# smacke/ffsubsync

Measured on AMD Instinct MI355X. Metric: alignments/sec (2 h@100 Hz, 7 framerate ratios), higher is better.
Workload: dtype i32; 1 GPU; configs[2]: 8192 x 7200 s@100 Hz pairs per GPU (8 batches of 1024), MaxScoreAligner over 7 framerate ratios, max_offset_samples=6000; algorithm=auto, pairs_per_gpu=8192, pairs_in_flight=512, n_fft_reference=2097152, n_fft_device=786432, input_format=bit-packed 0/1 vectors (FFS_DTYPE_U1) resident in HBM, parallelism=single GPU

## Files before the change

ffsubsync_amd/csrc/ffs_runs.h:

```cpp
#pragma once
#include "ffs_kernels.h"

namespace ffsa {

#ifndef FFS_RUNS_THREADS
#define FFS_RUNS_THREADS 512
#define FFS_RUNS_T 12288
#define FFS_RUNS_QCAP 3070
#endif
constexpr int RUNS_THREADS = FFS_RUNS_THREADS;
constexpr int RUNS_WAVES = RUNS_THREADS / 64;
constexpr int RUNS_T = FFS_RUNS_T;
constexpr int RUNS_LPT = RUNS_T / RUNS_THREADS;
constexpr int RUNS_QCAP = FFS_RUNS_QCAP;
static_assert(RUNS_T % RUNS_THREADS == 0 && RUNS_LPT % 4 == 0 && RUNS_LPT <= 32, "whole groups of four lags per thread, 32-bit edge windows");
constexpr int RUNS_CAP = 32768;
#ifndef FFS_RUNS_TPW
#define FFS_RUNS_TPW 2
#endif
constexpr int RUNS_TPW = FFS_RUNS_TPW;
constexpr int RUNS_QSENT = 0x1fffffff;
static_assert(RUNS_LPT <= 32 && RUNS_LPT % 4 == 0 && RUNS_QCAP % 2 == 0, "one 32-bit mask per thread, 8-byte histogram loads");

struct RunsRef {
    const int2* e;
    const int2* hdr;
    const unsigned* bits;
    int32_t len;
    int32_t cap;
};

struct RunEntry {
    int pos, ones;
};
typedef const __attribute__((address_space(1))) RunEntry* GEntries;
typedef const __attribute__((address_space(1))) int* GInts;
typedef const __attribute__((address_space(1))) unsigned* GWords;

struct RunsBest {
    double score;
    int32_t d;
    int32_t pad;
};

struct PackVec {
    const unsigned char* src;
    unsigned* dst;
    int32_t len;
    int32_t pad;
};

__global__ __launch_bounds__(256) void k_pack_bytes_batch(const PackVec* __restrict__ vecs, int chunks_per_vec) {
    const int v = blockIdx.x / chunks_per_vec, c = blockIdx.x - v * chunks_per_vec;
    const PackVec pv = vecs[v];
    const long long n = pv.len;
    const long long w = (long long)c * 256 + threadIdx.x;
    const long long n_words = (n + 31) >> 5;
    if (w >= n_words) return;
    const long long i0 = w * 32;
    const unsigned char* __restrict__ p = pv.src + i0;
    unsigned out = 0;
    if (i0 + 32 <= n) {
        unsigned wd[8];
        __builtin_memcpy(wd, p, 32);
#pragma unroll
        for (int k = 0; k < 8; ++k) {
            const unsigned t = nz_flags(wd[k]) >> 7;
            out |= (((t * 0x00204081u) >> 21) & 0xfu) << (4 * k);
        }
    } else {
        for (int k = 0; k < 32 && i0 + k < n; ++k) out |= (unsigned)(p[k] != 0) << k;
    }
    pv.dst[w] = out;
}

FFS_HD bool runs_over_budget(long long n_p, long long n_q, long long cap_p, long long cap_q, long long W, long long R, long long budget) {
    if (n_p >= cap_p || n_q >= cap_q) return true;
    const long long pairs = n_p * n_q;
    return pairs * W / (R > 0 ? R : 1) > budget;
}

FFS_DEV unsigned wave_incl_scan_u32(unsigned v) {
#define FFS_DPP_ADD(ctrl, rows) v += (unsigned)__builtin_amdgcn_update_dpp(0, (int)v, ctrl, rows, 0xf, false)
    FFS_DPP_ADD(0x111, 0xf);
    FFS_DPP_ADD(0x112, 0xf);
    FFS_DPP_ADD(0x114, 0xf);
    FFS_DPP_ADD(0x118, 0xf);
    FFS_DPP_ADD(0x142, 0xa);
    FFS_DPP_ADD(0x143, 0xc);
#undef FFS_DPP_ADD
    return v;
}

FFS_DEV float wave_max_f32(float v) {
#define FFS_DPP_MAX(ctrl, rows) v = fmaxf(v, __int_as_float(__builtin_amdgcn_update_dpp(__float_as_int(v), __float_as_int(v), ctrl, rows, 0xf, false)))
    FFS_DPP_MAX(0x111, 0xf);
    FFS_DPP_MAX(0x112, 0xf);
    FFS_DPP_MAX(0x114, 0xf);
    FFS_DPP_MAX(0x118, 0xf);
    FFS_DPP_MAX(0x142, 0xa);
    FFS_DPP_MAX(0x143, 0xc);
#undef FFS_DPP_MAX
    return __int_as_float(__builtin_amdgcn_readlane(__float_as_int(v), 63));
}

constexpr int RUNS_XQ = 256;
template <int NT>
FFS_DEV void runs_extract_lds(unsigned (*&s_e)[NT / 64 * 2], unsigned (*&s_o)[NT / 64 * 2], uint4 (*&s_q)[RUNS_XQ]) {
    __shared__ unsigned l_e[2][NT / 64 * 2], l_o[2][NT / 64 * 2];
    __shared__ __attribute__((aligned(16))) uint4 l_q[NT / 64][RUNS_XQ];
    s_e = l_e, s_o = l_o, s_q = l_q;
}
template <int NT, bool compact = false>
FFS_DEV void runs_extract_body(const unsigned* __restrict__ w_generic, const int len, int2* __restrict__ e, int2* __restrict__ hdr,
                               const int cap) {
    constexpr int NWV = NT / 64;
    constexpr int G = 2, SWEEP = NT * 4 * G;
    const int tid = threadIdx.x, lane = tid & 63, wave = __builtin_amdgcn_readfirstlane(tid >> 6);
    const gptr eb = (gptr)e;
    const int nw = (len + 31) >> 5;
    const int n_proc = (len >> 5) + 1;
    const unsigned tail = (len & 31) ? ((1u << (len & 31)) - 1u) : 0xffffffffu;
    unsigned(*s_e)[NWV * 2], (*s_o)[NWV * 2];
    uint4(*s_q)[RUNS_XQ];
    runs_extract_lds<NT>(s_e, s_o, s_q);
    uint4* const ring = s_q[wave];
    unsigned q_head = 0, q_tail = 0;
    unsigned n_bound = 0, n_ones = 0;
    unsigned xn[G][4], pn[G];
    const __amdgpu_buffer_rsrc_t vrs = __builtin_amdgcn_make_buffer_rsrc(const_cast<unsigned*>(w_generic), 0, nw * 4, 0x00020000);
    auto request = [&](int base) {
#pragma unroll
        for (int g = 0; g < G; ++g) {
            const int w0 = base + (g * NT + tid) * 4;
            typedef unsigned v4u __attribute__((ext_vector_type(4)));
            const v4u t = __builtin_amdgcn_raw_buffer_load_b128(vrs, w0 * 4, 0, 2);
            xn[g][0] = t.x, xn[g][1] = t.y, xn[g][2] = t.z, xn[g][3] = t.w;
            pn[g] = 0;
            if (lane == 0) pn[g] = __builtin_amdgcn_raw_buffer_load_b32(vrs, w0 * 4 - 4, 0, 0);
        }
    };
    auto drain = [&]() {
        const unsigned n = (q_tail - q_head) < 64u ? (q_tail - q_head) : 64u;
        if ((unsigned)lane < n) {
            const uint4 it = ring[(q_head + (unsigned)lane) & (RUNS_XQ - 1)];
            unsigned eb_k = it.y ^ __builtin_amdgcn_alignbit(it.y, it.x, 31);
            const int pos0 = (int)((it.x & 0x7fffffffu) << 5);
            int k_out = (int)it.w;
            while (eb_k) {
                const int b = __builtin_ctz(eb_k);
                if (k_out < cap) {
                    typedef int v2i __attribute__((ext_vector_type(2)));
                    if (compact)
                        *(__attribute__((address_space(1))) int*)(eb + 4u * (unsigned)k_out) = pos0 + b;
                    else
                        *(__attribute__((address_space(1))) v2i*)(eb + 8u * (unsigned)k_out) =
                            (v2i){pos0 + b, (int)it.z + (int)__popc(it.y & ((1u << b) - 1u))};
                }
                ++k_out;
                eb_k &= eb_k - 1;
            }
        }
        q_head += n;
    };
    request(0);
    int buf = 0;
    for (int base = 0; base < n_proc && n_bound < (unsigned)cap; base += SWEEP, buf ^= 1) {
        unsigned x[G][4], pv[G];
#pragma unroll
        for (int g = 0; g < G; ++g) {
            pv[g] = pn[g];
#pragma unroll
            for (int k = 0; k < 4; ++k) x[g][k] = xn[g][k];
            const int w0 = base + (g * NT + tid) * 4;
            if ((unsigned)(nw - 1 - w0) < 4u) {
#pragma unroll
                for (int k = 0; k < 4; ++k)
                    if (w0 + k == nw - 1) x[g][k] &= tail;
            }
            if (w0 == nw) pv[g] &= tail;
        }
        while (q_tail - q_head >= 64u) drain();
        if (base + SWEEP < n_proc) request(base + SWEEP);
        unsigned ne[G], no[G], pc = 0;
        unsigned fr[G];
#pragma unroll
        for (int g = 0; g < G; ++g) {
            unsigned prev = (unsigned)__builtin_amdgcn_update_dpp(0, (int)x[g][3], 0x138, 0xf, 0xf, false);
            if (lane == 0) prev = pv[g];
            fr[g] = prev;
            unsigned nc = 0;
            ne[g] = no[g] = 0;
#pragma unroll
            for (int k = 0; k < 4; ++k) {
                const unsigned e_k = x[g][k] ^ __builtin_amdgcn_alignbit(x[g][k], prev, 31);
                prev = x[g][k];
                ne[g] += __popc(e_k);
                no[g] += __popc(x[g][k]);
                nc += e_k != 0u ? 1u : 0u;
            }
            pc |= nc << (16 * g);
        }
        const unsigned ic = wave_incl_scan_u32(pc);
        unsigned qe = 0, qo = 0, se = 0, so = 0;
        unsigned ie[G], io[G];
        if (NT <= 256) {
            static_assert(G == 2, "two groups per packed scan");
            const unsigned pe = ne[0] | (ne[1] << 16), po = no[0] | (no[1] << 16);
            const unsigned je = wave_incl_scan_u32(pe), jo = wave_incl_scan_u32(po);
            if (lane == 63) s_e[buf][wave] = je, s_o[buf][wave] = jo;
            __syncthreads();
            qe = je - pe, qo = jo - po;
#pragma unroll
            for (int i = 0; i < NWV; ++i) {
                const unsigned a = s_e[buf][i], b = s_o[buf][i];
                if (i < wave) qe += a, qo += b;
                se += a, so += b;
            }
        } else {
#pragma unroll
            for (int g = 0; g < G; ++g) {
                ie[g] = wave_incl_scan_u32(ne[g]), io[g] = wave_incl_scan_u32(no[g]);
                if (lane == 63) s_e[buf][wave * G + g] = ie[g], s_o[buf][wave * G + g] = io[g];
                ie[g] -= ne[g], io[g] -= no[g];
            }
            __syncthreads();
        }
        const unsigned wc = (unsigned)__builtin_amdgcn_readlane((int)ic, 63);
        const unsigned rc = ic - pc;
        unsigned gb = n_bound, go = n_ones;
#pragma unroll
        for (int g = 0; g < G; ++g) {
            unsigned xe_g, xo_g, te_g = 0, to_g = 0;
            if (NT <= 256) {
                xe_g = (qe >> (16 * g)) & 0xffffu, xo_g = (qo >> (16 * g)) & 0xffffu, te_g = (se >> (16 * g)) & 0xffffu, to_g = (so >> (16 * g)) & 0xffffu;
            } else {
                xe_g = ie[g], xo_g = io[g];
                for (int i = 0; i < NWV; ++i) {
                    const unsigned a = s_e[buf][i * G + g], b = s_o[buf][i * G + g];
                    if (i < wave) xe_g += a, xo_g += b;
                    te_g += a, to_g += b;
                }
            }
            unsigned k_out = gb + xe_g;
            unsigned ones = go + xo_g;
            gb += te_g;
            go += to_g;
            const unsigned add = (wc >> (16 * g)) & 0xffffu;
            {
            while (q_tail - q_head + add > (unsigned)RUNS_XQ) drain();
            unsigned slot = q_tail + ((rc >> (16 * g)) & 0xffffu);
            const unsigned w0 = (unsigned)(base + (g * NT + tid) * 4);
            unsigned prev = fr[g];
#pragma unroll
            for (int k = 0; k < 4; ++k) {
                const unsigned e_k = x[g][k] ^ __builtin_amdgcn_alignbit(x[g][k], prev, 31);
                if (e_k) {
                    ring[slot & (RUNS_XQ - 1)] = make_uint4((w0 + k) | (prev & 0x80000000u), x[g][k], ones, k_out);
                    ++slot;
                }
                k_out += __popc(e_k);
                ones += __popc(x[g][k]);
                prev = x[g][k];
            }
            q_tail += add;
            asm volatile("s_waitcnt lgkmcnt(0)" ::: "memory");
            }
        }
        n_bound = gb, n_ones = go;
    }
    while (q_tail != q_head) drain();
    if (tid == 0) {
        *hdr = make_int2((int)n_bound, (int)n_ones);
        if ((int)n_bound < cap) {
            if (compact)
                reinterpret_cast<int*>(e)[n_bound] = INT32_MAX;
            else
                e[n_bound] = make_int2(INT32_MAX, (int)n_ones);
        }
    }
}

constexpr int RUNS_PROBE_WORDS = 256;
__global__ __launch_bounds__(256) void k_runs_probe(const RunsRef* __restrict__ refs, int n_vec) {
    const int v = blockIdx.x * 4 + (threadIdx.x >> 6), lane = threadIdx.x & 63;
    if (v >= n_vec) return;
    const RunsRef r = refs[v];
    if (!r.bits) return;
    const GWords w = (GWords)r.bits;
    const int nw = r.len >> 5;
    unsigned cnt = 0;
    if (nw > 0) {
#pragma unroll
        for (int u = 0; u < RUNS_PROBE_WORDS / 64; ++u) {
            const long long k = ((long long)(u * 64 + lane) * nw) / RUNS_PROBE_WORDS;
            const unsigned x = w[k];
            cnt += __popc((x ^ (x << 1)) & 0xfffffffeu);
        }
    }
#pragma unroll
    for (int s = 32; s >= 1; s >>= 1) cnt += __shfl_xor(cnt, s, 64);
    if (lane == 0) {
        const long long sampled = (long long)(nw < RUNS_PROBE_WORDS ? (nw > 0 ? nw : 1) : RUNS_PROBE_WORDS) * 31;
        long long est = (long long)cnt * (long long)r.len / sampled;
        if (est > 0x3fffffff) est = 0x3fffffff;
        const_cast<int2*>(r.hdr)[0] = make_int2((int)est, 0);
    }
}

FFS_DEV void runs_extract_zero(int* __restrict__ zero, int zero_words) {
    if (zero && blockIdx.x == 0)
        for (int i = threadIdx.x; i < zero_words; i += blockDim.x) zero[i] = 0;
}
FFS_DEV bool runs_compact_vec(int cstride, int n_plain) {
    return cstride > 0 && (int)blockIdx.x < n_plain && (int)blockIdx.x % cstride != 0;
}
__global__ __launch_bounds__(256, 8) void k_runs_extract(const RunsRef* __restrict__ refs, int* __restrict__ zero, int zero_words,
                                                         int cstride, int n_plain) {
    runs_extract_zero(zero, zero_words);
    const RunsRef r = refs[blockIdx.x];
    if (!r.bits) return;
    if (runs_compact_vec(cstride, n_plain))
        runs_extract_body<256, true>(r.bits, r.len, const_cast<int2*>(r.e), const_cast<int2*>(r.hdr), r.cap);
    else
        runs_extract_body<256, false>(r.bits, r.len, const_cast<int2*>(r.e), const_cast<int2*>(r.hdr), r.cap);
}
__global__ __launch_bounds__(512, 4) void k_runs_extract_512(const RunsRef* __restrict__ refs, int with_len_cap, int* __restrict__ zero,
                                                             int zero_words, int cstride, int n_plain) {
    runs_extract_zero(zero, zero_words);
    const RunsRef r = refs[blockIdx.x];
    if (!r.bits) return;
    if (with_len_cap && threadIdx.x == 0) const_cast<int2*>(r.hdr)[1] = make_int2(r.len, r.cap);
    if (runs_compact_vec(cstride, n_plain))
        runs_extract_body<512, true>(r.bits, r.len, const_cast<int2*>(r.e), const_cast<int2*>(r.hdr), r.cap);
    else
        runs_extract_body<512, false>(r.bits, r.len, const_cast<int2*>(r.e), const_cast<int2*>(r.hdr), r.cap);
}
__global__ __launch_bounds__(1024, 4) void k_runs_extract_1024(const RunsRef* __restrict__ refs, int with_len_cap, int* __restrict__ zero,
                                                               int zero_words, int cstride, int n_plain) {
    runs_extract_zero(zero, zero_words);
    const RunsRef r = refs[blockIdx.x];
    if (!r.bits) return;
    if (with_len_cap && threadIdx.x == 0) const_cast<int2*>(r.hdr)[1] = make_int2(r.len, r.cap);
    if (runs_compact_vec(cstride, n_plain))
        runs_extract_body<1024, true>(r.bits, r.len, const_cast<int2*>(r.e), const_cast<int2*>(r.hdr), r.cap);
    else
        runs_extract_body<1024, false>(r.bits, r.len, const_cast<int2*>(r.e), const_cast<int2*>(r.hdr), r.cap);
}

__global__ __launch_bounds__(256, 8) void k_runs_extract_lists(const RunsRef* __restrict__ refs) {
    const RunsRef r = refs[blockIdx.x];
    if (threadIdx.x == 0) const_cast<int2*>(r.hdr)[1] = make_int2(r.len, r.cap);
    runs_extract_body<256>(r.bits, r.len, const_cast<int2*>(r.e), const_cast<int2*>(r.hdr), r.cap);
}

__global__ __launch_bounds__(1024, 4) void k_runs_extract_one(const unsigned* __restrict__ bits, int len, int2* __restrict__ e,
                                                             int2* __restrict__ hdr, int cap) {
    if (threadIdx.x == 0) hdr[1] = make_int2(len, cap);
    runs_extract_body<1024>(bits, len, e, hdr, cap);
}

static inline void runs_extract_launch(const RunsRef* refs, size_t n_vec, bool with_len_cap, hipStream_t st, int* zero = nullptr,
                                       int zero_words = 0, int cstride = 0, int n_plain = 0) {
    if (with_len_cap) cstride = 0;
    if (n_vec <= 256)
        hipLaunchKernelGGL(k_runs_extract_1024, dim3((unsigned)n_vec), dim3(1024), 0, st, refs, with_len_cap ? 1 : 0, zero, zero_words, cstride, n_plain);
    else if (n_vec <= 768)
        hipLaunchKernelGGL(k_runs_extract_512, dim3((unsigned)n_vec), dim3(512), 0, st, refs, with_len_cap ? 1 : 0, zero, zero_words, cstride, n_plain);
    else if (with_len_cap)
        hipLaunchKernelGGL(k_runs_extract_lists, dim3((unsigned)n_vec), dim3(256), 0, st, refs);
    else
        hipLaunchKernelGGL(k_runs_extract, dim3((unsigned)n_vec), dim3(256), 0, st, refs, zero, zero_words, cstride, n_plain);
}

FFS_DEV unsigned fetch32(GWords w, int len, long long start) {
    const int nw = (len + 31) >> 5;
    const long long wi = start >> 5;
    unsigned v[2];
#pragma unroll
    for (int k = 0; k < 2; ++k) {
        const long long i = wi + k;
        unsigned t = (i >= 0 && i < nw) ? w[i] : 0u;
        if (i == nw - 1 && (len & 31)) t &= (1u << (len & 31)) - 1u;
        v[k] = t;
    }
    return __builtin_amdgcn_alignbit(v[1], v[0], (unsigned)(start & 31));
}

FFS_DEV unsigned list_bits32(GEntries e, int n, long long start) {
    if (start + 32 <= 0 || n <= 0) return 0u;
    int lo = 0, hi = n;
    while (lo < hi) {
        const int mid = (lo + hi) >> 1;
        if ((long long)e[mid].pos <= start)
            lo = mid + 1;
        else
            hi = mid;
    }
    unsigned m = (lo & 1) ? 0xffffffffu : 0u;
    for (int k = lo; k < n; ++k) {
        const long long off = (long long)e[k].pos - start;
        if (off >= 32) break;
        m ^= 0xffffffffu << (int)off;
    }
    return m;
}

FFS_DEV int wave_lower_bound_e(GEntries a, int n, int x) {
    const int lane = threadIdx.x & 63;
    int lo = 0, len = n;
    while (len > 0) {
        const int step = (len + 63) >> 6;
        const int idx = lo + (lane + 1) * step - 1;
        const bool below = idx < lo + len && a[idx].pos < x;
        const int c = __popcll(__ballot(below));
        const int end = lo + len;
        lo += c * step;
        len = (step - 1) < (end - lo) ? (step - 1) : (end - lo);
    }
    return lo;
}

template <int NW>
FFS_DEV void block_excl_scan3(int& a, int& b, int& c, int* s_tmp) {
    const int lane = threadIdx.x & 63, wave = threadIdx.x >> 6;
    int ia = a, ib = b, ic = c;
#pragma unroll
    for (int s = 1; s < 64; s <<= 1) {
        const int oa = __shfl_up(ia, s, 64), ob = __shfl_up(ib, s, 64), oc = __shfl_up(ic, s, 64);
        if (lane >= s) ia += oa, ib += ob, ic += oc;
    }
    __syncthreads();
    if (lane == 63) s_tmp[wave * 3] = ia, s_tmp[wave * 3 + 1] = ib, s_tmp[wave * 3 + 2] = ic;
    __syncthreads();
    int pa = ia - a, pb = ib - b, pc = ic - c;
#pragma unroll
    for (int i = 0; i < NW - 1; ++i)
        if (i < wave) pa += s_tmp[i * 3], pb += s_tmp[i * 3 + 1], pc += s_tmp[i * 3 + 2];
    a = pa, b = pb, c = pc;
}

constexpr int RUNS_FLAG_SPLIT = 8;
static inline unsigned runs_flag_split(long long cands_per_chunk) {
    const long long want = (cands_per_chunk + 447) / 448;
    return (unsigned)(want < RUNS_FLAG_SPLIT ? RUNS_FLAG_SPLIT : (want > 128 ? 128 : want));
}
__global__ __launch_bounds__(256) void k_runs_chunk_flags(const CandDesc* __restrict__ cands, int n_pairs, int n_cand,
                                                          int pairs_per_chunk, const RunsRef* __restrict__ refs, long long budget,
                                                          int* __restrict__ flags, unsigned long long* __restrict__ stats,
                                                          int estimates) {
    const int ch = blockIdx.x;
    const int p0 = ch * pairs_per_chunk, p1 = (p0 + pairs_per_chunk) < n_pairs ? (p0 + pairs_per_chunk) : n_pairs;
    int over = 0, bad = 0;
    unsigned long long nb = 0;
    int longest = 0;
    for (int i = p0 * n_cand + (int)(blockIdx.y * 256 + threadIdx.x); i < p1 * n_cand; i += 256 * (int)gridDim.y) {
        const CandDesc& cd = cands[i];
        const int pair = i / n_cand, j = i - pair * n_cand;
        const int vr = pair * (n_cand + 1), vs = vr + 1 + j;
        const RunsRef rr = refs[vr], rs = refs[vs];
        const GInts hq = (GInts)rr.hdr, hp = (GInts)rs.hdr;
        const int n_q = hq[0], n_p = hp[0];
        const int cap_q = (estimates && rr.bits) ? 0x7fffffff : (rr.cap > 0 ? rr.cap : hq[3]);
        const int cap_p = (estimates && rs.bits) ? 0x7fffffff : (rs.cap > 0 ? rs.cap : hp[3]);
        nb += (unsigned)n_p + (j == 0 ? (unsigned)n_q : 0u);
        if (rs.bits && n_p > longest) longest = n_p;
        if (rr.bits && n_q > longest) longest = n_q;
        bad |= (!rs.bits && n_p >= cap_p) || (!rr.bits && n_q >= cap_q);
        if (cd.flags & CAND_NO_LAGS) continue;
        const int lim_q = (estimates && rr.bits) ? cap_q : (cap_q < RUNS_CAP ? cap_q : RUNS_CAP);
        const int lim_p = (estimates && rs.bits) ? cap_p : (cap_p < RUNS_CAP ? cap_p : RUNS_CAP);
        over |= runs_over_budget(n_p, n_q, lim_p, lim_q, (long long)cd.d_hi - cd.d_lo + 1, cd.R, budget) ? 1 : 0;
    }
    over = __syncthreads_or(over);
    bad = __syncthreads_or(bad);
    __shared__ unsigned long long s_nb[4];
#pragma unroll
    for (int s = 32; s >= 1; s >>= 1) nb += __shfl_xor(nb, s, 64);
    if ((threadIdx.x & 63) == 0) s_nb[threadIdx.x >> 6] = nb;
    __syncthreads();
    if (threadIdx.x == 0) {
        const int f = bad ? 2 : over;
        if (f) atomicMax(&flags[ch], f);
        if (!estimates) atomicAdd(stats, s_nb[0] + s_nb[1] + s_nb[2] + s_nb[3]);
    }
    if (!estimates) {
#pragma unroll
        for (int s = 32; s >= 1; s >>= 1) {
            const int o = __shfl_xor(longest, s, 64);
            longest = o > longest ? o : longest;
        }
        if ((threadIdx.x & 63) == 0 && longest > 0) atomicMax(stats + 1, (unsigned long long)longest);
    }
}

FFS_DEV void runs_write_cand(const CandDesc& cd, CandResult* __restrict__ cres, int ci, double score, int d, bool none) {
    CandResult r;
    if (none) {
        r.score = -INFINITY;
        r.offset = (long long)cd.n_ref - 1 - cd.S;
        r.score_f32 = -INFINITY;
        r.flags = 1;
    } else {
        r.score = score;
        r.offset = d;
        r.score_f32 = (float)score;
        r.flags = 0;
    }
    apply_zero_rule(cd, r);
    cres[ci] = r;
}

struct LevelInfo {
    double lam[4];
    double q;
    int32_t n_levels;
    int32_t m[3];
    int32_t ok;
    int32_t pad[3];
};
constexpr int LEVELS_MAX_MULT = 8;

template <class T>
FFS_DEV void levels_insert(double (&v)[5], int& n, T x) {
    const double d = (double)x;
    bool seen = false;
#pragma unroll
    for (int i = 0; i < 5; ++i) seen |= (i < n && v[i] == d);
    if (!seen && n < 5) {
#pragma unroll
        for (int i = 0; i < 5; ++i)
            if (i == n) v[i] = d;
        ++n;
    }
}

template <class T>
__global__ __launch_bounds__(256) void k_levels_sample(const T* const* __restrict__ vec, const int* __restrict__ len, LevelInfo* __restrict__ out) {
    const int v = blockIdx.x, tid = threadIdx.x, lane = tid & 63, wave = tid >> 6;
    typedef const __attribute__((address_space(1))) T* GT;
    const GT x = (GT)vec[v];
    const int n = len[v];
    double vals[5] = {0.0, 0.0, 0.0, 0.0, 0.0};
    int cnt = 0;
#pragma unroll
    for (int u = 0; u < 8; ++u) {
        const long long k = ((long long)(u * 256 + tid) * n) / 2048;
        if (k < n) levels_insert(vals, cnt, x[k]);
    }
    __shared__ double s_v[4][5];
    __shared__ int s_n[4];
    for (int s = 1; s < 64; s <<= 1) {
        const int cn = __shfl_xor(cnt, s, 64);
        double pv[5];
#pragma unroll
        for (int i = 0; i < 5; ++i) pv[i] = __shfl_xor(vals[i], s, 64);
#pragma unroll
        for (int i = 0; i < 5; ++i)
            if (i < cn) levels_insert(vals, cnt, pv[i]);
    }
    double (&wv)[5] = vals;
    const int wn = cnt;
    if (lane == 0) {
        s_n[wave] = wn;
#pragma unroll
        for (int i = 0; i < 5; ++i) s_v[wave][i] = wv[i];
    }
    __syncthreads();
    if (tid == 0) {
        double all[5];
        int an = 0;
        for (int w = 0; w < 4; ++w)
            for (int i = 0; i < s_n[w] && i < 5; ++i) levels_insert(all, an, s_v[w][i]);
        for (int i = 1; i < an && i < 5; ++i)
// ... 921 lines not shown
```

Before: 2.701 million 7-ratio solves/s.

## Stage run-boundary records in an LDS window and flush coalesced line-aligned stores

Boundary records produced by the run-extraction kernel are no longer written straight to global memory from the drain loop. Each sweep's records go into an LDS window, and the whole block then flushes them with line-aligned, coalesced stores at the start of the next sweep. The point is to replace scattered per-lane global writes with contiguous cache-line writes. The cost is extra LDS, a full queue drain every sweep, an extra synchronisation, and a fallback to direct stores when a sweep's records exceed the window. It also adds compile-time A/B switches for isolating store cost.

```diff
diff --git a/ffsubsync_amd/csrc/ffs_runs.h b/ffsubsync_amd/csrc/ffs_runs.h
--- a/ffsubsync_amd/csrc/ffs_runs.h
+++ b/ffsubsync_amd/csrc/ffs_runs.h
@@ -106,27 +106,38 @@
 
 constexpr int RUNS_XQ = 256;
 template <int NT>
-FFS_DEV void runs_extract_lds(unsigned (*&s_e)[NT / 64 * 2], unsigned (*&s_o)[NT / 64 * 2], uint4 (*&s_q)[RUNS_XQ]) {
+constexpr int runs_xwin_bytes() {
+    return NT == 256 ? 496 * 8 : NT * 16;
+}
+template <int NT>
+FFS_DEV void runs_extract_lds(unsigned (*&s_e)[NT / 64 * 2], unsigned (*&s_o)[NT / 64 * 2], uint4 (*&s_q)[RUNS_XQ], unsigned*& s_win) {
     __shared__ unsigned l_e[2][NT / 64 * 2], l_o[2][NT / 64 * 2];
     __shared__ __attribute__((aligned(16))) uint4 l_q[NT / 64][RUNS_XQ];
-    s_e = l_e, s_o = l_o, s_q = l_q;
+    __shared__ __attribute__((aligned(8))) unsigned l_win[runs_xwin_bytes<NT>() / 4];
+    s_e = l_e, s_o = l_o, s_q = l_q, s_win = l_win;
 }
 template <int NT, bool compact = false>
 FFS_DEV void runs_extract_body(const unsigned* __restrict__ w_generic, const int len, int2* __restrict__ e, int2* __restrict__ hdr,
                                const int cap) {
     constexpr int NWV = NT / 64;
     constexpr int G = 2, SWEEP = NT * 4 * G;
+    constexpr unsigned ES = compact ? 4u : 8u;
+    constexpr unsigned WIN = runs_xwin_bytes<NT>() / ES;
+    constexpr unsigned LINE = 128u / ES;
     const int tid = threadIdx.x, lane = tid & 63, wave = __builtin_amdgcn_readfirstlane(tid >> 6);
     const gptr eb = (gptr)e;
+    const unsigned mis = ((unsigned)(size_t)e / ES) & (LINE - 1u);
     const int nw = (len + 31) >> 5;
     const int n_proc = (len >> 5) + 1;
     const unsigned tail = (len & 31) ? ((1u << (len & 31)) - 1u) : 0xffffffffu;
     unsigned(*s_e)[NWV * 2], (*s_o)[NWV * 2];
     uint4(*s_q)[RUNS_XQ];
-    runs_extract_lds<NT>(s_e, s_o, s_q);
+    unsigned* s_win;
+    runs_extract_lds<NT>(s_e, s_o, s_q, s_win);
     uint4* const ring = s_q[wave];
     unsigned q_head = 0, q_tail = 0;
     unsigned n_bound = 0, n_ones = 0;
+    unsigned st_lo = 0, w_org = 0;
     unsigned xn[G][4], pn[G];
     const __amdgpu_buffer_rsrc_t vrs = __builtin_amdgcn_make_buffer_rsrc(const_cast<unsigned*>(w_generic), 0, nw * 4, 0x00020000);
     auto request = [&](int base) {
@@ -140,22 +151,58 @@
             if (lane == 0) pn[g] = __builtin_amdgcn_raw_buffer_load_b32(vrs, w0 * 4 - 4, 0, 0);
         }
     };
-    auto drain = [&]() {
+#if defined(FFS_EXTRACT_AB) && FFS_EXTRACT_AB == 1
+    unsigned ab_sink = 0;
+#endif
+    auto put = [&](unsigned k, int pos, int ones) {
+#if defined(FFS_EXTRACT_AB) && FFS_EXTRACT_AB == 1
+        ab_sink += k + (unsigned)pos + (unsigned)ones;
+#else
+#if defined(FFS_EXTRACT_AB) && FFS_EXTRACT_AB == 2
+        if (cap < 64) return;
+        k &= 63u;
+#endif
+        typedef int v2i __attribute__((ext_vector_type(2)));
+        if (compact)
+            *(__attribute__((address_space(1))) int*)(eb + 4u * k) = pos;
+        else
+            *(__attribute__((address_space(1))) v2i*)(eb + 8u * k) = (v2i){pos, ones};
+#endif
+    };
+    auto slot_of = [&](unsigned k, unsigned org) {
+        const unsigned s = k - org;
+        return s < s - WIN ? s : s - WIN;
+    };
+    auto flush = [&](unsigned lo, unsigned hi, unsigned org) {
+        if (hi > (unsigned)cap) hi = (unsigned)cap;
+        for (int k = (int)lo - (int)((lo + mis) & (LINE - 1u)) + tid; k < (int)hi; k += NT)
+            if (k >= (int)lo) {
+                const unsigned s = slot_of((unsigned)k, org);
+                if (compact) {
+                    put((unsigned)k, (int)s_win[s], 0);
+                } else {
+                    const uint2 v = reinterpret_cast<const uint2*>(s_win)[s];
+                    put((unsigned)k, (int)v.x, (int)v.y);
+                }
+            }
+    };
+    auto drain = [&](const bool stage) {
         const unsigned n = (q_tail - q_head) < 64u ? (q_tail - q_head) : 64u;
         if ((unsigned)lane < n) {
             const uint4 it = ring[(q_head + (unsigned)lane) & (RUNS_XQ - 1)];
             unsigned eb_k = it.y ^ __builtin_amdgcn_alignbit(it.y, it.x, 31);
             const int pos0 = (int)((it.x & 0x7fffffffu) << 5);
-            int k_out = (int)it.w;
+            unsigned k_out = it.w;
             while (eb_k) {
                 const int b = __builtin_ctz(eb_k);
-                if (k_out < cap) {
-                    typedef int v2i __attribute__((ext_vector_type(2)));
-                    if (compact)
-                        *(__attribute__((address_space(1))) int*)(eb + 4u * (unsigned)k_out) = pos0 + b;
+                if (k_out < (unsigned)cap) {
+                    const int pos = pos0 + b, ones = (int)it.z + (int)__popc(it.y & ((1u << b) - 1u));
+                    if (!stage)
+                        put(k_out, pos, ones);
+                    else if (compact)
+                        s_win[slot_of(k_out, w_org)] = (unsigned)pos;
                     else
-                        *(__attribute__((address_space(1))) v2i*)(eb + 8u * (unsigned)k_out) =
-                            (v2i){pos0 + b, (int)it.z + (int)__popc(it.y & ((1u << b) - 1u))};
+                        reinterpret_cast<uint2*>(s_win)[slot_of(k_out, w_org)] = make_uint2((unsigned)pos, (unsigned)ones);
                 }
                 ++k_out;
                 eb_k &= eb_k - 1;
@@ -180,8 +227,6 @@
             }
             if (w0 == nw) pv[g] &= tail;
         }
-        while (q_tail - q_head >= 64u) drain();
-        if (base + SWEEP < n_proc) request(base + SWEEP);
         unsigned ne[G], no[G], pc = 0;
         unsigned fr[G];
 #pragma unroll
@@ -204,6 +249,7 @@
         const unsigned ic = wave_incl_scan_u32(pc);
         unsigned qe = 0, qo = 0, se = 0, so = 0;
         unsigned ie[G], io[G];
+        unsigned cnt;
         if (NT <= 256) {
             static_assert(G == 2, "two groups per packed scan");
             const unsigned pe = ne[0] | (ne[1] << 16), po = no[0] | (no[1] << 16);
@@ -217,6 +263,7 @@
                 if (i < wave) qe += a, qo += b;
                 se += a, so += b;
             }
+            cnt = (se & 0xffffu) + (se >> 16);
         } else {
 #pragma unroll
             for (int g = 0; g < G; ++g) {
@@ -225,7 +272,16 @@
                 ie[g] -= ne[g], io[g] -= no[g];
             }
             __syncthreads();
-        }
+            cnt = (unsigned)__builtin_amdgcn_readlane((int)wave_incl_scan_u32(lane < NWV * G ? s_e[buf][lane] : 0u), 63);
+        }
+        flush(st_lo, n_bound, w_org);
+        if (base + SWEEP < n_proc) request(base + SWEEP);
+        const bool stage = n_bound - st_lo + cnt <= WIN;
+        st_lo = stage ? n_bound : n_bound + cnt;
+        if (!stage)
+            w_org = st_lo;
+        else if (st_lo - w_org >= WIN)
+            w_org += WIN;
         const unsigned wc = (unsigned)__builtin_amdgcn_readlane((int)ic, 63);
         const unsigned rc = ic - pc;
         unsigned gb = n_bound, go = n_ones;
@@ -247,8 +303,8 @@
             gb += te_g;
             go += to_g;
             const unsigned add = (wc >> (16 * g)) & 0xffffu;
-            {
-            while (q_tail - q_head + add > (unsigned)RUNS_XQ) drain();
+            if (q_tail - q_head + add > (unsigned)RUNS_XQ)
+                while (q_tail != q_head) drain(stage);
             unsigned slot = q_tail + ((rc >> (16 * g)) & 0xffffu);
             const unsigned w0 = (unsigned)(base + (g * NT + tid) * 4);
             unsigned prev = fr[g];
@@ -265,11 +321,15 @@
             }
             q_tail += add;
             asm volatile("s_waitcnt lgkmcnt(0)" ::: "memory");
-            }
-        }
+        }
+        while (q_tail != q_head) drain(stage);
         n_bound = gb, n_ones = go;
     }
-    while (q_tail != q_head) drain();
+    __syncthreads();
+    flush(st_lo, n_bound, w_org);
+#if defined(FFS_EXTRACT_AB) && FFS_EXTRACT_AB == 1
+    if (ab_sink == 0x9e3779b9u && len < 0) hdr[0].y = (int)ab_sink;
+#endif
     if (tid == 0) {
         *hdr = make_int2((int)n_bound, (int)n_ones);
         if ((int)n_bound < cap) {
```

New measurement: 2.724 million 7-ratio solves/s (median of 6 runs). No clear change (+0.8%).
